# twice154/ofa-for-super-resolution

Hardware: AMD Instinct MI355X
Metric: sr_training_images_per_sec_4x_64to256 (higher is better)
Workload: dtype bf16; 1 GPU; OFA-SR S4 supernet 4x progressive shrinking (elastic kernel {3,5,7}, e=6, d=4, pd=2), LR 64x64 -> HR 256x256, fwd+bwd+Adam, train-mode BN; kernel_transform_mode=1, compat_reference_indexing=True, parallelism=dp1, per_gpu_batch=16, global_batch=16, grad_allreduce_bytes=0, launch=eager

## Files before the change

### ofa-for-super-resolution_amd/csrc/dwconv.hip

```cpp
#include "ofasr_common.h"

#include <type_traits>

namespace ofasr {

constexpr int DW_WAVES = 4;

template <int D>
__device__ __forceinline__ float lane_shift(float v, int lane) {
    if (D == 0) return v;
    const int src = lane + D;
    const float t = __shfl(v, src & 63, 64);
    return (src >= 0 && src < 64) ? t : 0.f;
}

template <int K>
struct Strips {
    static constexpr int PAD = K / 2;
    static __host__ __device__ int count(int W) { return W <= 64 ? 1 : (W + (64 - 2 * PAD) - 1) / (64 - 2 * PAD); }
    static __device__ int col0(int W, int s) { return W <= 64 ? 0 : s * (64 - 2 * PAD) - PAD; }
    static __device__ bool core(int W, int lane) { return W <= 64 ? true : (lane >= PAD && lane < 64 - PAD); }
};

template <typename T, int K, bool FLIP>
__global__ void __launch_bounds__(64 * DW_WAVES) dw_strip_kernel(const T* __restrict__ x, const float* __restrict__ f,
                                                                 T* __restrict__ y, int C, int H, int W,
                                                                 int nstrips, int nchunks, int rows_per_chunk,
                                                                 long long units) {
    constexpr int PAD = K / 2;
    const int lane = lane_id();
    const int wave = __builtin_amdgcn_readfirstlane((int)(threadIdx.x >> 6));
    const long long unit = (long long)blockIdx.x * DW_WAVES + wave;
    if (unit >= units) return;
    const int chunk = (int)(unit % nchunks);
// ... 201 lines not shown

template <typename T, int K> struct VecPx { static constexpr int N = (K <= 3 && sizeof(T) == 2) ? 8 : 4; };

template <int PXL, int PAD>
__device__ __forceinline__ void build_window(const float* v, float* win, int lane, bool has_left, bool has_right) {
#pragma unroll
    for (int i = 0; i < PAD; ++i) {
        const float l = __shfl(v[PXL - PAD + i], (lane + 63) & 63, 64);
        const float r = __shfl(v[i], (lane + 1) & 63, 64);
        win[i] = has_left ? l : 0.f;
        win[PAD + PXL + i] = has_right ? r : 0.f;
    }
#pragma unroll
    for (int i = 0; i < PXL; ++i) win[PAD + i] = v[i];
}

typedef __attribute__((ext_vector_type(16))) float dwm_f32x16;
typedef __attribute__((ext_vector_type(8))) short dwm_s16x8;
typedef __attribute__((ext_vector_type(8))) __bf16 dwm_bf16x8;
typedef __attribute__((ext_vector_type(8))) _Float16 dwm_f16x8;
template <typename T> struct DwMma;
template <> struct DwMma<bf16_t> {
    static __device__ __forceinline__ dwm_f32x16 run(dwm_s16x8 a, dwm_s16x8 b, dwm_f32x16 c) {
        return __builtin_amdgcn_mfma_f32_32x32x16_bf16(__builtin_bit_cast(dwm_bf16x8, a), __builtin_bit_cast(dwm_bf16x8, b),
                                                       c, 0, 0, 0);
    }
};
template <> struct DwMma<f16_t> {
    static __device__ __forceinline__ dwm_f32x16 run(dwm_s16x8 a, dwm_s16x8 b, dwm_f32x16 c) {
        return __builtin_amdgcn_mfma_f32_32x32x16_f16(__builtin_bit_cast(dwm_f16x8, a), __builtin_bit_cast(dwm_f16x8, b), c,
                                                      0, 0, 0);
    }
};
constexpr int DWM_NPW = 4;
constexpr int DWM_PITCH = 144;
__device__ __forceinline__ void dwm_lds_fence() { asm volatile("s_waitcnt lgkmcnt(0)" ::: "memory"); }

template <typename T, int K, bool FLIP, bool XF, bool STAT, bool BX = false>
__global__ void __launch_bounds__(64 * DW_WAVES) dw_mfma_kernel(const T* __restrict__ x, const float* __restrict__ f,
                                                                T* __restrict__ y, int N, int C, int H, int W,
                                                                int nslabs, InputXf xf, StatOut so, BnFold fold,
                                                                BwdXf bx = BwdXf{}) {
    constexpr int PAD = K / 2;
    constexpr int LROWS = 64 + 2 * PAD;
    __shared__ __attribute__((aligned(16))) char planes[DW_WAVES][LROWS * DWM_PITCH];
    __shared__ __attribute__((aligned(16))) char outs[DW_WAVES][64 * 128];
    __shared__ uint16_t tapt[DW_WAVES][K][96];
    const int lane = lane_id();
    const int wave = __builtin_amdgcn_readfirstlane((int)(threadIdx.x >> 6));
    const long long unit = (long long)blockIdx.x * DW_WAVES + wave;
    const int c = (int)(unit % C);
    const int n0 = (int)(unit / C) * DWM_NPW;
    if (n0 >= N) return;
    char* L = planes[wave];
    const int r = lane & 31, hh = lane >> 5;

    for (int i = lane; i < LROWS * (DWM_PITCH / 16); i += 64) *reinterpret_cast<uint4*>(L + i * 16) = make_uint4(0, 0, 0, 0);
    for (int i = lane; i < K * 96; i += 64) tapt[wave][i / 96][i % 96] = 0;
    dwm_lds_fence();
    for (int e = lane; e < K * K; e += 64)
        tapt[wave][e / K][e % K + 40] = from_float<T>(f[(long long)c * K * K + (FLIP ? (K * K - 1 - e) : e)]).v;
    dwm_lds_fence();
    dwm_s16x8 Bf[K][3];
#pragma unroll
    for (int ky = 0; ky < K; ++ky)
#pragma unroll
        for (int ch = 0; ch < 3; ++ch) {
            const int base = (-8 + 16 * ch) + 8 * hh - r + PAD + 40;
            dwm_s16x8 b;
#pragma unroll
            for (int i = 0; i < 8; ++i) b[i] = (short)tapt[wave][ky][base + i];
            Bf[ky][ch] = b;
        }

    float xsc = 1.f, xmu = 0.f, xb = 0.f;
    if constexpr (XF) {
        if (fold.cp) {
            double s = 0.0, ss = 0.0;
            for (int q0 = lane; q0 < fold.P; q0 += 8 * 64) {
                float2 v[8];
#pragma unroll
                for (int j = 0; j < 8; ++j) {
                    const int q = q0 + 64 * j < fold.P ? q0 + 64 * j : fold.P - 1;
                    v[j] = fold.cp[(long long)c * fold.P + q];
                }
#pragma unroll
                for (int j = 0; j < 8; ++j) {
                    const bool live = q0 + 64 * j < fold.P;
                    s += live ? (double)v[j].x : 0.0;
                    ss += live ? (double)v[j].y : 0.0;
                }
            }
#pragma unroll
            for (int o = 32; o > 0; o >>= 1) {
                s += __shfl_xor(s, o, 64);
                ss += __shfl_xor(ss, o, 64);
            }
            const double mean = s / fold.M;
            double var = ss / fold.M - mean * mean;
            var = var < 0.0 ? 0.0 : var;
            const double invstd = 1.0 / sqrt(var + fold.eps);
            const double gm = fold.gamma ? (double)fold.gamma[c] : 1.0, bt = fold.beta ? (double)fold.beta[c] : 0.0;
            xsc = (float)(gm * invstd);
            xmu = (float)mean;
            xb = (float)bt;
            if (n0 == 0 && lane == 0) {
                fold.mean[c] = (float)mean;
                fold.invstd[c] = (float)invstd;
                fold.scale[c] = xsc;
                fold.shift[c] = (float)(bt - mean * gm * invstd);
                if (fold.running_mean) {
                    const double unb = fold.M > 1.0 ? var * fold.M / (fold.M - 1.0) : var;
                    fold.running_mean[c] =
                        (float)((1.0 - fold.momentum) * (double)fold.running_mean[c] + fold.momentum * mean);
                    fold.running_var[c] = (float)((1.0 - fold.momentum) * (double)fold.running_var[c] + fold.momentum * unb);
                }
                if (c == 0) {
#pragma unroll
                    for (int i = 0; i < 3; ++i)
                        if (fold.counters[i]) *fold.counters[i] += 1;
                }
            }
        } else {
            xsc = xf.scale[c];
            xmu = xf.mean[c];
            xb = fmaf(xmu, xsc, xf.shift[c]);
        }
    }

    float bmu = 0.f, bsc = 1.f, bxb = 0.f, bka = 0.f, bkbi = 0.f;
    if constexpr (BX) {
        bmu = bx.mean[c];
        bsc = bx.scale[c];
        bxb = fmaf(bmu, bsc, bx.shift[c]);
        if (bx.fold_partial) bwdxf_fold(bx, c, bsc, n0 == 0 && lane == 0, bka, bkbi);
        else {
            bka = bx.ka[c];
            bkbi = bx.kbi[c];
        }
    }

    int abase[2][3];
#pragma unroll
    for (int wb = 0; wb < 2; ++wb)
#pragma unroll
        for (int ch = 0; ch < 3; ++ch) {
            const int cidx = 4 * wb - 1 + 2 * ch + hh;
            const int cz = (cidx < 0 || cidx >= (W >> 3)) ? 8 : cidx;
            abase[wb][ch] = r * DWM_PITCH + cz * 16;
        }
    const int cpr = W >> 3;
    const int nchunks = H * cpr;
    char* O = outs[wave];
    uint4 nxt[8];
    uint4 nxt2[BX ? 8 : 1];
    auto load_plane = [&](int pl) {
        const long long plane = (long long)(n0 + pl) * C + c;
        const uint4* src = reinterpret_cast<const uint4*>(x + plane * (long long)H * W);
#pragma unroll
        for (int it = 0; it < 8; ++it) {
            const int idx = lane + 64 * it;
            nxt[it] = src[idx < nchunks ? idx : 0];
        }
        if constexpr (BX) {
            const uint4* src2 = reinterpret_cast<const uint4*>(reinterpret_cast<const T*>(bx.y) + plane * (long long)H * W);
#pragma unroll
            for (int it = 0; it < 8; ++it) {
                const int idx = lane + 64 * it;
                nxt2[it] = src2[idx < nchunks ? idx : 0];
            }
        }
    };
    load_plane(0);
    for (int pl = 0; pl < DWM_NPW && n0 + pl < N; ++pl) {
        const long long plane = (long long)(n0 + pl) * C + c;
#pragma unroll
        for (int it = 0; it < 8; ++it) {
            const int idx = lane + 64 * it;
            if (idx < nchunks) {
                uint4 v = nxt[it];
                if constexpr (XF) {
                    uint32_t wv[4] = {v.x, v.y, v.z, v.w};
#pragma unroll
                    for (int i = 0; i < 4; ++i) {
                        T lo, hi;
                        lo.v = (uint16_t)(wv[i] & 0xffffu);
                        hi.v = (uint16_t)(wv[i] >> 16);
                        const float a = fminf(fmaxf(fmaf(to_float(lo) - xmu, xsc, xb), 0.f), 6.f);
                        const float b = fminf(fmaxf(fmaf(to_float(hi) - xmu, xsc, xb), 0.f), 6.f);
                        wv[i] = pack2<T>(a, b);
                    }
                    v = make_uint4(wv[0], wv[1], wv[2], wv[3]);
                }
                if constexpr (BX) {
                    uint32_t wv[4] = {v.x, v.y, v.z, v.w};
                    const uint32_t yv[4] = {nxt2[it].x, nxt2[it].y, nxt2[it].z, nxt2[it].w};
#pragma unroll
                    for (int i = 0; i < 4; ++i) {
                        T lo, hi, ylo, yhi;
                        lo.v = (uint16_t)(wv[i] & 0xffffu);
                        hi.v = (uint16_t)(wv[i] >> 16);
                        ylo.v = (uint16_t)(yv[i] & 0xffffu);
                        yhi.v = (uint16_t)(yv[i] >> 16);
                        const float t0 = to_float(ylo) - bmu, t1 = to_float(yhi) - bmu;
                        const float p0 = fmaf(t0, bsc, bxb), p1 = fmaf(t1, bsc, bxb);
                        const float z0 = (p0 > 0.f && p0 < 6.f) ? to_float(lo) : 0.f;
                        const float z1 = (p1 > 0.f && p1 < 6.f) ? to_float(hi) : 0.f;
                        wv[i] = pack2<T>(fmaf(-t0, bkbi, fmaf(bsc, z0, -bka)), fmaf(-t1, bkbi, fmaf(bsc, z1, -bka)));
                    }
                    v = make_uint4(wv[0], wv[1], wv[2], wv[3]);
                    if (bx.dy_out)
                        reinterpret_cast<uint4*>(reinterpret_cast<T*>(bx.dy_out) + plane * (long long)H * W)[idx] = v;
                }
                const int row = idx / cpr, chunk = idx - row * cpr, lr = row + PAD;
                *reinterpret_cast<uint4*>(L + lr * DWM_PITCH + (chunk << 4)) = v;
            }
        }
        dwm_lds_fence();
        if (pl + 1 < DWM_NPW && n0 + pl + 1 < N) load_plane(pl + 1);
        float st_s = 0.f, st_q = 0.f;
        for (int hb = 0; hb < H / 32; ++hb) {
            const char* Lh = L + hb * (32 * DWM_PITCH);
#pragma unroll
            for (int wb = 0; wb < 2; ++wb) {
                if (32 * wb >= W) break;
                dwm_f32x16 acc;
#pragma unroll
                for (int i = 0; i < 16; ++i) acc[i] = 0.f;
#pragma unroll
                for (int ky = 0; ky < K; ++ky) {
#pragma unroll
                    for (int ch = 0; ch < 3; ++ch) {
                        const dwm_s16x8 a =
                            *reinterpret_cast<const dwm_s16x8*>(Lh + abase[wb][ch] + ky * DWM_PITCH);
                        acc = DwMma<T>::run(Bf[ky][ch], a, acc);
                    }
                }
                const int h = 32 * hb + r;
#pragma unroll
                for (int q = 0; q < 4; ++q) {
                    const uint2 o = make_uint2(pack2<T>(acc[4 * q], acc[4 * q + 1]), pack2<T>(acc[4 * q + 2], acc[4 * q + 3]));
                    const int chunk = 4 * wb + q;
                    *reinterpret_cast<uint2*>(O + h * 128 + ((chunk ^ ((h >> 1) & 7)) << 4) + 8 * hh) = o;
                    if constexpr (STAT) {
                        const uint32_t wv2[2] = {o.x, o.y};
#pragma unroll
                        for (int i = 0; i < 2; ++i) {
                            T lo, hi;
                            lo.v = (uint16_t)(wv2[i] & 0xffffu);
                            hi.v = (uint16_t)(wv2[i] >> 16);
                            const float a0 = to_float(lo), a1 = to_float(hi);
                            st_s += a0 + a1;
                            st_q = fmaf(a0, a0, fmaf(a1, a1, st_q));
                        }
                    }
                }
            }
        }
        dwm_lds_fence();
        uint4* dst = reinterpret_cast<uint4*>(y + plane * (long long)H * W);
#pragma unroll
        for (int it = 0; it < 8; ++it) {
            const int idx = lane + 64 * it;
            if (idx < nchunks) {
                const int row = idx / cpr, chunk = idx - row * cpr;
                dst[idx] = *reinterpret_cast<const uint4*>(O + row * 128 + ((chunk ^ ((row >> 1) & 7)) << 4));
            }
        }
        dwm_lds_fence();
        if constexpr (STAT) {
            const float s = wave_sum(st_s), q = wave_sum(st_q);
            if (lane == 0) {
                so.partial[(long long)c * so.P + (long long)(n0 + pl) * nslabs] = make_float2(s, q);
                for (int sl = 1; sl < nslabs; ++sl)
                    so.partial[(long long)c * so.P + (long long)(n0 + pl) * nslabs + sl] = make_float2(0.f, 0.f);
            }
        }
    }
}

static bool mfma_geom_ok(int64_t H, int64_t W, int K, const void* a, const void* b) {
    const uintptr_t bits = reinterpret_cast<uintptr_t>(a) | reinterpret_cast<uintptr_t>(b);
    return K >= 5 && (W == 32 || W == 64) && H >= 32 && H <= 64 && (H % 32) == 0 && (bits & 15) == 0;
}

struct VecGeom {
    int G, gpw, R, nslabs;
};

template <typename T, int K, bool FLIP, bool XF = false, bool STAT = false, bool BX = false>
__global__ void __launch_bounds__(64 * DW_WAVES) dw_vec_kernel(const T* __restrict__ x, const float* __restrict__ f,
                                                               T* __restrict__ y, int C, int H, int W, VecGeom vg,
                                                               long long nwaves, InputXf xf = InputXf{},
                                                               StatOut so = StatOut{nullptr, 0}, BnFold fold = BnFold{},
                                                               BwdXf bx = BwdXf{}) {
    constexpr int PAD = K / 2;
    constexpr int PXL = VecPx<T, K>::N;
    typedef PxIO<T, PXL> IO;
    typedef typename IO::raw_t raw_t;
    const int lane = lane_id();
    const int wave = __builtin_amdgcn_readfirstlane((int)(threadIdx.x >> 6));
    const long long wunit = (long long)blockIdx.x * DW_WAVES + wave;
    if (wunit >= nwaves) return;
    const int slab = (int)(wunit % vg.nslabs);
    const long long plane = wunit / vg.nslabs;
    const int c = (int)(plane % C);

    float taps[K * K];
#pragma unroll
    for (int e = 0; e < K * K; ++e) taps[e] = f[(long long)c * K * K + (FLIP ? (K * K - 1 - e) : e)];
    float bmu = 0.f, bsc = 1.f, bxb = 0.f, bka = 0.f, bkbi = 0.f;
    if constexpr (BX) {
        bmu = bx.mean[c];
        bsc = bx.scale[c];
        bxb = fmaf(bmu, bsc, bx.shift[c]);
        if (bx.fold_partial) bwdxf_fold(bx, c, bsc, plane < C && slab == 0 && lane == 0, bka, bkbi);
// ... 271 lines not shown
    vg.G = (int)(W / PXL);
    vg.gpw = 64 / vg.G;
    int64_t R = cdiv(H, vg.gpw);
    if (R < 4) R = 4;
    if (R > 32) R = 32;
    vg.R = (int)R;
    vg.nslabs = (int)cdiv(H, (int64_t)vg.gpw * vg.R);
    return true;
}

__global__ void __launch_bounds__(256) dw_wgrad_reduce_kernel(const float* __restrict__ part_out,
                                                              float* __restrict__ df, int nparts, long long CKK) {
    const long long idx = (long long)blockIdx.x * blockDim.x + threadIdx.x;
    if (idx >= CKK) return;
    float s = 0.f;
    for (int p = 0; p < nparts; ++p) s += part_out[(long long)p * CKK + idx];
    df[idx] = s;
}

static int wgrad_parts(int64_t N, int64_t C) {
    int64_t want = cdiv(6144, C > 0 ? C : 1);
    if (want < 1) want = 1;
    if (want > N) want = N;
    return (int)want;
}

template <typename T, bool FLIP, bool XF = false, bool STAT = false, bool BX = false>
static int launch_conv(const char* name, const void* x, const float* f, void* y, int64_t N, int64_t C, int64_t H,
                       int64_t W, int K, hipStream_t st, InputXf xf = InputXf{}, StatOut so = StatOut{nullptr, 0},
                       BnFold fold = BnFold{}, BwdXf bx = BwdXf{}) {
    prof_note(2.0 * sizeof(T) * (double)N * (double)C * (double)H * (double)W + 4.0 * (double)C * K * K,
              2.0 * K * K * (double)N * (double)C * (double)H * (double)W);
    if constexpr (sizeof(T) == 2) {
        if (mfma_geom_ok(H, W, K, x, y)) {
            VecGeom vg0;
            const int nslabs = vec_geom(H, W, 2, 4, x, y, vg0) ? vg0.nslabs : 1;
            if (STAT && so.P != (int)(N * nslabs)) {
                set_error("%s: statistics slab count %d != %lld", name, so.P, (long long)(N * nslabs));
                return OFASR_ERR_INVALID_ARG;
            }
            const long long units = (long long)C * cdiv(N, DWM_NPW);
            if (K == 5)
                OFASR_LAUNCH((dw_mfma_kernel<T, 5, FLIP, XF, STAT, BX>), dim3((unsigned)cdiv(units, DW_WAVES)),
                                   dim3(64 * DW_WAVES), 0, st, (const T*)x, f, (T*)y, (int)N, (int)C, (int)H, (int)W, nslabs,
                                   xf, so, fold, bx);
            else
                OFASR_LAUNCH((dw_mfma_kernel<T, 7, FLIP, XF, STAT, BX>), dim3((unsigned)cdiv(units, DW_WAVES)),
                                   dim3(64 * DW_WAVES), 0, st, (const T*)x, f, (T*)y, (int)N, (int)C, (int)H, (int)W, nslabs,
                                   xf, so, fold, bx);
            return check_launch(name);
        }
    }
    {
        VecGeom vg;
#define OFASR_DWV(KK)                                                                                               \
    if (vec_geom(H, W, (int)sizeof(T), VecPx<T, KK>::N, x, y, vg)) {                                               \
        const long long nwaves = (long long)N * C * vg.nslabs;                                                     \
        if (STAT && so.P != (int)(N * vg.nslabs)) {                                                                \
            set_error("%s: statistics slab count %d != %lld", name, so.P, (long long)(N * vg.nslabs));             \
            return OFASR_ERR_INVALID_ARG;                                                                          \
        }                                                                                                          \
        OFASR_LAUNCH((dw_vec_kernel<T, KK, FLIP, XF, STAT, BX>), dim3((unsigned)cdiv(nwaves, DW_WAVES)),     \
                           dim3(64 * DW_WAVES), 0, st, (const T*)x, f, (T*)y, (int)C, (int)H, (int)W, vg, nwaves,  \
                           xf, so, fold, bx);                                                                      \
        return check_launch(name);                                                                                 \
    }
        switch (K) {
            case 1: OFASR_DWV(1) break;
            case 3: OFASR_DWV(3) break;
            case 5: OFASR_DWV(5) break;
            default: OFASR_DWV(7) break;
        }
#undef OFASR_DWV
    }
    if constexpr (XF || BX) {
        set_error("%s: fused input transform needs the vector kernel", name);
        return OFASR_ERR_UNSUPPORTED;
    }
    const int rows_per_chunk = H <= 32 ? (int)H : 32;
    const int nchunks = (int)cdiv(H, rows_per_chunk);
#define OFASR_DW_LAUNCH(KK)                                                                                  \
    {                                                                                                        \
// ... 435 lines not shown
```

### ofa-for-super-resolution_amd/csrc/conv2d.hip

```cpp
#include "ofasr_common.h"

namespace ofasr {

typedef __attribute__((ext_vector_type(16))) float cv_f32x16;
typedef __attribute__((ext_vector_type(8))) __bf16 cv_bf16x8;
typedef __attribute__((ext_vector_type(8))) _Float16 cv_f16x8;
typedef __attribute__((ext_vector_type(8))) short cv_s16x8;

constexpr int CV_TW = 64;
constexpr int CV_SEG = 20;
constexpr int CV_RP = 4 * CV_SEG;
constexpr int CV_KC = 32;

template <typename T> struct CvMma;
template <> struct CvMma<bf16_t> {
    static __device__ __forceinline__ cv_f32x16 run(cv_s16x8 a, cv_s16x8 b, cv_f32x16 c) {
        return __builtin_amdgcn_mfma_f32_32x32x16_bf16(__builtin_bit_cast(cv_bf16x8, a), __builtin_bit_cast(cv_bf16x8, b),
                                                       c, 0, 0, 0);
    }
};
template <> struct CvMma<f16_t> {
    static __device__ __forceinline__ cv_f32x16 run(cv_s16x8 a, cv_s16x8 b, cv_f32x16 c) {
        return __builtin_amdgcn_mfma_f32_32x32x16_f16(__builtin_bit_cast(cv_f16x8, a), __builtin_bit_cast(cv_f16x8, b), c,
                                                      0, 0, 0);
    }
};

__device__ __forceinline__ int cv_pos(int r, int col) { return r * CV_RP + (col & 3) * CV_SEG + (col >> 2); }
__device__ __forceinline__ int cv_rec(int P, int j) { return P * 64 + ((j ^ ((P >> 2) & 3)) << 4); }

struct CvBn {
    float* ss;
    const float* gamma;
// ... 476 lines not shown
    const int wq = wave % (WCO * WCI);
    if constexpr (WK > 1) {
        static_assert(WCO * WCI * RBW * 4096 <= ROWS * 256, "Yt holds one tx slice per (wco, wci)");
        float* red = reinterpret_cast<float*>(Yt) + wq * (RBW * 16 * 64) + lane;
#pragma unroll
        for (int tx = 0; tx < KS; ++tx) {
#pragma unroll
            for (int ph = 1; ph < WK; ++ph) {
                __syncthreads();
                if (wk == ph) {
#pragma unroll
                    for (int rb = 0; rb < RBW; ++rb)
#pragma unroll
                        for (int reg = 0; reg < 16; ++reg) red[(rb * 16 + reg) * 64] = acc[rb][tx][reg];
                }
                __syncthreads();
                if (wk == 0) {
#pragma unroll
                    for (int rb = 0; rb < RBW; ++rb)
#pragma unroll
                        for (int reg = 0; reg < 16; ++reg) acc[rb][tx][reg] += red[(rb * 16 + reg) * 64];
                }
            }
        }
        if (wk != 0) return;
    }
    float* dst = part + ((((long long)split * KS + ty) * P.nz + z) * (WCO * WCI) + wq) * (RBW * KS * 16 * 64) + lane;
#pragma unroll
    for (int rb = 0; rb < RBW; ++rb)
#pragma unroll
        for (int tx = 0; tx < KS; ++tx)
#pragma unroll
            for (int reg = 0; reg < 16; ++reg) dst[((rb * KS + tx) * 16 + reg) * 64] = acc[rb][tx][reg];
}

template <int KS, int RBW, int WCO, int WCI>
__global__ void __launch_bounds__(256) conv_wgrad_reduce_kernel(const float* __restrict__ part, float* __restrict__ dw,
                                                                CvWgParams P, long long total) {
    const long long idx = (long long)blockIdx.x * blockDim.x + threadIdx.x;
    if (idx >= total) return;
    constexpr int PER_WAVE = RBW * KS * 16 * 64;
    long long t = idx;
    const int lane = (int)(t & 63);
    t >>= 6;
    const int reg = (int)(t & 15);
    t >>= 4;
    const int tx = (int)(t % KS);
    t /= KS;
    const int rb = (int)(t % RBW);
    t /= RBW;
    const int wq = (int)(t % (WCO * WCI));
    t /= (WCO * WCI);
    const int z = (int)(t % P.nz);
    const int ty = (int)(t / P.nz);
    const int wco = wq % WCO, wci = wq / WCO;
    const int coslab = z / P.ncislab, cislab = z % P.ncislab;
    const int co = coslab * (32 * RBW * WCO) + 32 * (wco * RBW + rb) + (reg & 3) + 8 * (reg >> 2) + 4 * (lane >> 5);
    const int ci = cislab * (32 * WCI) + 32 * wci + (lane & 31);
    if (co >= P.Cout || ci >= P.Cin) return;
    const long long inner = ((long long)(rb * KS + tx) * 16 + reg) * 64 + lane;
    float sum = 0.f;
    const long long sstride = (long long)KS * P.nz * (WCO * WCI) * PER_WAVE;
    const float* src = part + (((long long)ty * P.nz + z) * (WCO * WCI) + wq) * PER_WAVE + inner;
    for (int split = 0; split < P.ksplit; ++split) sum += src[split * sstride];
    dw[(((long long)co * P.Cin + ci) * KS + ty) * KS + tx] = sum;
}
// ... 7 lines not shown
};

static CvWgPlan cv_wg_plan(int64_t N, int64_t Cin, int64_t Cout, int64_t H, int64_t W, int K) {
    CvWgPlan p{};
    p.note_bytes = 2.0 * (double)N * (double)H * (double)W * (double)(Cin + Cout);
    p.note_flops = 2.0 * (double)N * (double)H * (double)W * (double)Cin * (double)Cout * K * K;
    const bool wide = Cin > 32;
    const int rcls = Cout > 64 ? 0 : (Cout > 32 ? 1 : 2);
    p.cfg = (wide ? 0 : 3) + rcls;
    p.rows = rcls == 0 ? 128 : (rcls == 1 ? 64 : 32);
    p.rbw = rcls == 2 ? 1 : 2;
    p.cib = wide ? 64 : 32;
    CvWgParams& P = p.P;
    P.Cin = (int)Cin; P.Cout = (int)Cout; P.H = (int)H; P.W = (int)W;
    P.tiles_x = (int)cdiv(W, CV_TW); P.tiles_y = (int)cdiv(H, 2);
    P.ntiles = (int)(N * P.tiles_x * P.tiles_y);
    P.ncislab = (int)cdiv(Cin, p.cib);
    P.nz = (int)cdiv(Cout, p.rows) * P.ncislab;
    int ks = 512 / (K * P.nz);
    ks = ks > P.ntiles / 8 ? P.ntiles / 8 : ks;
    if (ks > 8) ks -= ks % 8;
    P.ksplit = ks < 1 ? 1 : ks;
    const int nwq = wide ? (rcls == 0 ? 4 : 2) : (rcls == 0 ? 2 : 1);
    p.part_bytes = (size_t)P.ksplit * K * P.nz * nwq * (p.rbw * K * 16 * 64) * sizeof(float);
    return p;
}

template <typename T>
static int launch_conv2d_wgrad(const char* name, const void* dy, const void* x, float* dw, int K, const CvWgPlan& p, void* ws,
                               hipStream_t st) {
    const CvWgParams& P = p.P;
    dim3 grid((unsigned)(cdiv(P.ksplit, 8) * 8 * K * P.nz));
    prof_note(p.note_bytes, p.note_flops);
#define OFASR_WG(KS, RBW, WCO, WCI, WK)                                                                              \
    {                                                                                                                \
        OFASR_LAUNCH((conv_wgrad_kernel<T, KS, RBW, WCO, WCI, WK>), grid, dim3(256), 0, st, (const T*)dy,      \
                           (const T*)x, (float*)ws, P);                                                              \
        int rc = check_launch(name);                                                                                 \
        if (rc) return rc;                                                                                           \
        const long long tot = (long long)KS * P.nz * (WCO * WCI) * RBW * KS * 16 * 64;                               \
        OFASR_LAUNCH((conv_wgrad_reduce_kernel<KS, RBW, WCO, WCI>), dim3((unsigned)cdiv(tot, 256)),            \
                           dim3(256), 0, st, (const float*)ws, dw, P, tot);                                          \
    }
#define OFASR_WGK(KS)                                                                                                \
    switch (p.cfg) {                                                                                                 \
        case 0: OFASR_WG(KS, 2, 2, 2, 1) break;                                                                      \
        case 1: OFASR_WG(KS, 2, 1, 2, 2) break;                                                                      \
        case 2: OFASR_WG(KS, 1, 1, 2, 2) break;                                                                      \
        case 3: OFASR_WG(KS, 2, 2, 1, 2) break;                                                                      \
        case 4: OFASR_WG(KS, 2, 1, 1, 4) break;                                                                      \
        default: OFASR_WG(KS, 1, 1, 1, 4) break;                                                                     \
    }
    if (K == 5) { OFASR_WGK(5) } else { OFASR_WGK(3) }
#undef OFASR_WGK
#undef OFASR_WG
    return check_launch(name);
}

static int conv_stat_units(int64_t N, int64_t Cin, int64_t Cout, int64_t H, int64_t W, int K) {
    if (conv_thin_out_supported(Cout, Cin, K, W, OFASR_BF16, nullptr, nullptr))
        return conv_thin_out_units(N, Cout, Cin, H, W, OFASR_BF16);
    if (conv_thin_in_supported(Cin, Cout, K, W, OFASR_BF16, nullptr, nullptr))
        return conv_thin_in_units(N, Cin, Cout, H, W, OFASR_BF16);
    const CvPlan p = cv_plan(Cin, Cout, K, 0, N, H, W);
    const int wp = p.th / 2;
    return (int)(N * cdiv(W, CV_TW) * cdiv(H, p.th) * wp);
}
// ... 155 lines not shown
```

Measured before the change: 2789 images/s.

## Adapt depthwise MFMA conv planes-per-wave to CU count with channel-contiguous work split

Replaces the fixed four-images-per-wave assignment of the MFMA depthwise conv with a plan that picks planes-per-wave from the CU count, so small N*C launches fill the GPU. Waves now walk a contiguous range of (channel, image) planes and may cross channels, so per-channel setup (taps, BN fold statistics, backward fold) moves into a re-entrant routine. That routine issues its global loads early and prefetches the first plane before the LDS setup. It also adds a waves-per-EU hint and an environment override. The cost is redundant per-channel fold reductions across more waves and more complex counter and writer logic.

New measurement: 2754 images/s. 0.987x the previous value.

```diff
diff --git a/ofa-for-super-resolution_amd/csrc/dw_fill.h b/ofa-for-super-resolution_amd/csrc/dw_fill.h
--- /dev/null
+++ b/ofa-for-super-resolution_amd/csrc/dw_fill.h
@@ -0,0 +1,55 @@
+#pragma once
+
+#if defined(__HIPCC__)
+#define OFASR_DWF_HD __host__ __device__ __forceinline__
+#else
+#define OFASR_DWF_HD inline
+#endif
+
+namespace ofasr {
+
+constexpr int DWF_MAX_PPW = 4;
+constexpr int DWF_WAVES_PER_SIMD = 2;
+constexpr int DWF_SIMDS_PER_CU = 4;
+
+struct DwFill {
+    int ppw;
+    int legacy;
+};
+
+OFASR_DWF_HD long long dwf_waves(int N, int C, DwFill pl) {
+    if (pl.legacy) return (long long)C * ((N + DWF_MAX_PPW - 1) / DWF_MAX_PPW);
+    return ((long long)N * C + pl.ppw - 1) / pl.ppw;
+}
+
+OFASR_DWF_HD void dwf_range(long long u, int N, int C, DwFill pl, int& p0, int& p1) {
+    const long long total = (long long)N * C;
+    long long a, b;
+    if (pl.legacy) {
+        const long long c = u % C, n0 = (u / C) * DWF_MAX_PPW;
+        a = c * N + (n0 < N ? n0 : N);
+        b = c * N + (n0 + DWF_MAX_PPW < N ? n0 + DWF_MAX_PPW : N);
+    } else {
+        a = u * pl.ppw;
+        b = a + pl.ppw;
+    }
+    if (u < 0 || a > total) a = total;
+    if (u < 0 || b > total) b = total;
+    p0 = (int)a;
+    p1 = (int)b;
+}
+
+OFASR_DWF_HD int dwf_channel(int p, int N) { return p / N; }
+OFASR_DWF_HD int dwf_image(int p, int N) { return p % N; }
+OFASR_DWF_HD bool dwf_is_writer(int p, int N) { return p % N == 0; }
+OFASR_DWF_HD bool dwf_owns_counters(int p) { return p == 0; }
+
+inline int dwf_choose_ppw(long long planes, long long slots) {
+    for (int ppw = 1; ppw < DWF_MAX_PPW; ++ppw)
+        if ((planes + ppw - 1) / ppw <= slots) return ppw;
+    return DWF_MAX_PPW;
+}
+
+inline long long dwf_slots(int cu_count) { return (long long)DWF_WAVES_PER_SIMD * DWF_SIMDS_PER_CU * cu_count; }
+
+}
diff --git a/ofa-for-super-resolution_amd/csrc/dwconv.hip b/ofa-for-super-resolution_amd/csrc/dwconv.hip
--- a/ofa-for-super-resolution_amd/csrc/dwconv.hip
+++ b/ofa-for-super-resolution_amd/csrc/dwconv.hip
@@ -1,5 +1,9 @@
 #include "ofasr_common.h"
-
+#include "dw_fill.h"
+
+#include <string.h>
+
+#include <atomic>
 #include <type_traits>
 
 namespace ofasr {
@@ -267,15 +271,14 @@
                                                       0, 0, 0);
     }
 };
-constexpr int DWM_NPW = 4;
 constexpr int DWM_PITCH = 144;
 __device__ __forceinline__ void dwm_lds_fence() { asm volatile("s_waitcnt lgkmcnt(0)" ::: "memory"); }
 
 template <typename T, int K, bool FLIP, bool XF, bool STAT, bool BX = false>
-__global__ void __launch_bounds__(64 * DW_WAVES) dw_mfma_kernel(const T* __restrict__ x, const float* __restrict__ f,
+__global__ void __launch_bounds__(64 * DW_WAVES) __attribute__((amdgpu_waves_per_eu(2))) dw_mfma_kernel(const T* __restrict__ x, const float* __restrict__ f,
                                                                 T* __restrict__ y, int N, int C, int H, int W,
-                                                                int nslabs, InputXf xf, StatOut so, BnFold fold,
-                                                                BwdXf bx = BwdXf{}) {
+                                                                int nslabs, DwFill plan, InputXf xf, StatOut so,
+                                                                BnFold fold, BwdXf bx = BwdXf{}) {
     constexpr int PAD = K / 2;
     constexpr int LROWS = 64 + 2 * PAD;
     __shared__ __attribute__((aligned(16))) char planes[DW_WAVES][LROWS * DWM_PITCH];
@@ -283,36 +286,120 @@
     __shared__ uint16_t tapt[DW_WAVES][K][96];
     const int lane = lane_id();
     const int wave = __builtin_amdgcn_readfirstlane((int)(threadIdx.x >> 6));
-    const long long unit = (long long)blockIdx.x * DW_WAVES + wave;
-    const int c = (int)(unit % C);
-    const int n0 = (int)(unit / C) * DWM_NPW;
-    if (n0 >= N) return;
+    int p0, p1;
+    dwf_range((long long)blockIdx.x * DW_WAVES + wave, N, C, plan, p0, p1);
+    if (p0 >= p1) return;
     char* L = planes[wave];
     const int r = lane & 31, hh = lane >> 5;
 
-    for (int i = lane; i < LROWS * (DWM_PITCH / 16); i += 64) *reinterpret_cast<uint4*>(L + i * 16) = make_uint4(0, 0, 0, 0);
-    for (int i = lane; i < K * 96; i += 64) tapt[wave][i / 96][i % 96] = 0;
-    dwm_lds_fence();
-    for (int e = lane; e < K * K; e += 64)
-        tapt[wave][e / K][e % K + 40] = from_float<T>(f[(long long)c * K * K + (FLIP ? (K * K - 1 - e) : e)]).v;
-    dwm_lds_fence();
+    int abase[2][3];
+#pragma unroll
+    for (int wb = 0; wb < 2; ++wb)
+#pragma unroll
+        for (int ch = 0; ch < 3; ++ch) {
+            const int cidx = 4 * wb - 1 + 2 * ch + hh;
+            const int cz = (cidx < 0 || cidx >= (W >> 3)) ? 8 : cidx;
+            abase[wb][ch] = r * DWM_PITCH + cz * 16;
+        }
+    const int cpr = W >> 3;
+    const int nchunks = H * cpr;
+    char* O = outs[wave];
+    uint4 nxt[8];
+    uint4 nxt2[BX ? 8 : 1];
+    auto load_plane = [&](int p) {
+        const long long plane = (long long)dwf_image(p, N) * C + dwf_channel(p, N);
+        const uint4* src = reinterpret_cast<const uint4*>(x + plane * (long long)H * W);
+        int ll = lane;
+        asm volatile("" : "+v"(ll));
+#pragma unroll
+        for (int it = 0; it < 8; ++it) {
+            const int idx = ll + 64 * it;
+            nxt[it] = src[idx < nchunks ? idx : 0];
+        }
+        if constexpr (BX) {
+            const uint4* src2 = reinterpret_cast<const uint4*>(reinterpret_cast<const T*>(bx.y) + plane * (long long)H * W);
+#pragma unroll
+            for (int it = 0; it < 8; ++it) {
+                const int idx = ll + 64 * it;
+                nxt2[it] = src2[idx < nchunks ? idx : 0];
+            }
+        }
+    };
     dwm_s16x8 Bf[K][3];
-#pragma unroll
-    for (int ky = 0; ky < K; ++ky)
-#pragma unroll
-        for (int ch = 0; ch < 3; ++ch) {
-            const int base = (-8 + 16 * ch) + 8 * hh - r + PAD + 40;
-            dwm_s16x8 b;
-#pragma unroll
-            for (int i = 0; i < 8; ++i) b[i] = (short)tapt[wave][ky][base + i];
-            Bf[ky][ch] = b;
-        }
-
     float xsc = 1.f, xmu = 0.f, xb = 0.f;
+    float bmu = 0.f, bsc = 1.f, bxb = 0.f, bka = 0.f, bkbi = 0.f;
+    constexpr bool EARLY = !BX;
+    auto enter_channel = [&](const int c, const bool writer, const bool counters, const bool first, const int p_first) {
+    static_assert(K * K <= 64, "one tap per lane");
+    int ln = lane;
+    asm volatile("" : "+v"(ln));
+    const int te = ln < K * K ? ln : 0;
+    const float tapv = f[(long long)c * K * K + (FLIP ? (K * K - 1 - te) : te)];
+    float2 v0[8];
+    float gmv = 1.f, btv = 0.f, rmv = 0.f, rvv = 0.f;
+    long long cnt[3] = {0, 0, 0};
+    if constexpr (XF) {
+        if (fold.cp) {
+#pragma unroll
+            for (int j = 0; j < 8; ++j) {
+                const int q = ln + 64 * j < fold.P ? ln + 64 * j : fold.P - 1;
+                v0[j] = fold.cp[(long long)c * fold.P + q];
+            }
+            if (fold.gamma) gmv = fold.gamma[c];
+            if (fold.beta) btv = fold.beta[c];
+            if (fold.running_mean) {
+                rmv = fold.running_mean[c];
+                rvv = fold.running_var[c];
+            }
+            if (counters) {
+#pragma unroll
+                for (int i = 0; i < 3; ++i)
+                    if (fold.counters[i]) cnt[i] = *fold.counters[i];
+            }
+        } else {
+            xsc = xf.scale[c];
+            xmu = xf.mean[c];
+            xb = xf.shift[c];
+        }
+    }
+    double fa[8], fb[8];
+    float bsh = 0.f, binv = 0.f;
+    if constexpr (BX) {
+        bmu = bx.mean[c];
+        bsc = bx.scale[c];
+        bsh = bx.shift[c];
+        if (bx.fold_partial) {
+            binv = bx.fold_invstd[c];
+#pragma unroll
+            for (int j = 0; j < 8; ++j) {
+                const int q = j < bx.fold_P ? j : bx.fold_P - 1;
+                fa[j] = bx.fold_partial[((long long)q * bx.fold_C + c) * 2];
+                fb[j] = bx.fold_partial[((long long)q * bx.fold_C + c) * 2 + 1];
+            }
+        } else {
+            bka = bx.ka[c];
+            bkbi = bx.kbi[c];
+        }
+    }
+    if constexpr (EARLY)
+        if (first) load_plane(p_first);
+    __builtin_amdgcn_sched_barrier(0);
+
+    if (first) {
+        for (int i = ln; i < LROWS * (DWM_PITCH / 16); i += 64) *reinterpret_cast<uint4*>(L + i * 16) = make_uint4(0, 0, 0, 0);
+        for (int i = ln; i < K * 96; i += 64) tapt[wave][i / 96][i % 96] = 0;
+        dwm_lds_fence();
+    }
     if constexpr (XF) {
         if (fold.cp) {
             double s = 0.0, ss = 0.0;
-            for (int q0 = lane; q0 < fold.P; q0 += 8 * 64) {
+#pragma unroll
+            for (int j = 0; j < 8; ++j) {
+                const bool live = ln + 64 * j < fold.P;
+                s += live ? (double)v0[j].x : 0.0;
+                ss += live ? (double)v0[j].y : 0.0;
+            }
+            for (int q0 = ln + 8 * 64; q0 < fold.P; q0 += 8 * 64) {
                 float2 v[8];
 #pragma unroll
                 for (int j = 0; j < 8; ++j) {
@@ -335,80 +422,92 @@
             double var = ss / fold.M - mean * mean;
             var = var < 0.0 ? 0.0 : var;
             const double invstd = 1.0 / sqrt(var + fold.eps);
-            const double gm = fold.gamma ? (double)fold.gamma[c] : 1.0, bt = fold.beta ? (double)fold.beta[c] : 0.0;
+            const double gm = fold.gamma ? (double)gmv : 1.0, bt = fold.beta ? (double)btv : 0.0;
             xsc = (float)(gm * invstd);
             xmu = (float)mean;
             xb = (float)bt;
-            if (n0 == 0 && lane == 0) {
+            if (writer && lane == 0) {
                 fold.mean[c] = (float)mean;
                 fold.invstd[c] = (float)invstd;
                 fold.scale[c] = xsc;
                 fold.shift[c] = (float)(bt - mean * gm * invstd);
                 if (fold.running_mean) {
                     const double unb = fold.M > 1.0 ? var * fold.M / (fold.M - 1.0) : var;
-                    fold.running_mean[c] =
-                        (float)((1.0 - fold.momentum) * (double)fold.running_mean[c] + fold.momentum * mean);
-                    fold.running_var[c] = (float)((1.0 - fold.momentum) * (double)fold.running_var[c] + fold.momentum * unb);
-                }
-                if (c == 0) {
+                    fold.running_mean[c] = (float)((1.0 - fold.momentum) * (double)rmv + fold.momentum * mean);
+                    fold.running_var[c] = (float)((1.0 - fold.momentum) * (double)rvv + fold.momentum * unb);
+                }
+                if (counters) {
 #pragma unroll
                     for (int i = 0; i < 3; ++i)
-                        if (fold.counters[i]) *fold.counters[i] += 1;
+                        if (fold.counters[i]) {
+                            long long bump = 1;
+                            for (int j = 0; j < i; ++j) bump += fold.counters[j] == fold.counters[i] ? 1 : 0;
+                            *fold.counters[i] = cnt[i] + bump;
+                        }
                 }
             }
         } else {
-            xsc = xf.scale[c];
-            xmu = xf.mean[c];
-            xb = fmaf(xmu, xsc, xf.shift[c]);
-        }
-    }
-
-    float bmu = 0.f, bsc = 1.f, bxb = 0.f, bka = 0.f, bkbi = 0.f;
+            xb = fmaf(xmu, xsc, xb);
+        }
+    }
+
     if constexpr (BX) {
-        bmu = bx.mean[c];
-        bsc = bx.scale[c];
-        bxb = fmaf(bmu, bsc, bx.shift[c]);
-        if (bx.fold_partial) bwdxf_fold(bx, c, bsc, n0 == 0 && lane == 0, bka, bkbi);
-        else {
-            bka = bx.ka[c];
-            bkbi = bx.kbi[c];
-        }
-    }
-
-    int abase[2][3];
-#pragma unroll
-    for (int wb = 0; wb < 2; ++wb)
+        bxb = fmaf(bmu, bsc, bsh);
+        if (bx.fold_partial) {
+            double s = 0.0, sx = 0.0;
+            asm volatile("" : "+v"(s), "+v"(sx), "+v"(binv));
+#pragma unroll
+            for (int j = 0; j < 8; ++j) {
+                s += j < bx.fold_P ? fa[j] : 0.0;
+                sx += j < bx.fold_P ? fb[j] : 0.0;
+            }
+            for (int q0 = 8; q0 < bx.fold_P; q0 += 8) {
+#pragma unroll
+                for (int j = 0; j < 8; ++j) {
+                    const int q = q0 + j < bx.fold_P ? q0 + j : bx.fold_P - 1;
+                    fa[j] = bx.fold_partial[((long long)q * bx.fold_C + c) * 2];
+                    fb[j] = bx.fold_partial[((long long)q * bx.fold_C + c) * 2 + 1];
+                }
+#pragma unroll
+                for (int j = 0; j < 8; ++j) {
+                    s += q0 + j < bx.fold_P ? fa[j] : 0.0;
+                    sx += q0 + j < bx.fold_P ? fb[j] : 0.0;
+                }
+            }
+            bka = bx.fold_training ? (float)((double)bsc * (s / bx.fold_M)) : 0.f;
+            bkbi = bx.fold_training ? (float)((double)bsc * (double)binv * (sx / bx.fold_M)) : 0.f;
+            if (writer && lane == 0) {
+                if (bx.fold_dgamma) bx.fold_dgamma[c] = (float)sx;
+                if (bx.fold_dbeta) bx.fold_dbeta[c] = (float)s;
+                if (bx.coef_ka) bx.coef_ka[c] = bka;
+                if (bx.coef_kbi) bx.coef_kbi[c] = bkbi;
+            }
+        }
+    }
+
+    if (ln < K * K) tapt[wave][ln / K][ln % K + 40] = from_float<T>(tapv).v;
+    dwm_lds_fence();
+#pragma unroll
+    for (int ky = 0; ky < K; ++ky)
 #pragma unroll
         for (int ch = 0; ch < 3; ++ch) {
-            const int cidx = 4 * wb - 1 + 2 * ch + hh;
-            const int cz = (cidx < 0 || cidx >= (W >> 3)) ? 8 : cidx;
-            abase[wb][ch] = r * DWM_PITCH + cz * 16;
-        }
-    const int cpr = W >> 3;
-    const int nchunks = H * cpr;
-    char* O = outs[wave];
-    uint4 nxt[8];
-    uint4 nxt2[BX ? 8 : 1];
-    auto load_plane = [&](int pl) {
-        const long long plane = (long long)(n0 + pl) * C + c;
-        const uint4* src = reinterpret_cast<const uint4*>(x + plane * (long long)H * W);
-#pragma unroll
-        for (int it = 0; it < 8; ++it) {
-            const int idx = lane + 64 * it;
-            nxt[it] = src[idx < nchunks ? idx : 0];
-        }
-        if constexpr (BX) {
-            const uint4* src2 = reinterpret_cast<const uint4*>(reinterpret_cast<const T*>(bx.y) + plane * (long long)H * W);
-#pragma unroll
-            for (int it = 0; it < 8; ++it) {
-                const int idx = lane + 64 * it;
-                nxt2[it] = src2[idx < nchunks ? idx : 0];
-            }
-        }
+            const int base = (-8 + 16 * ch) + 8 * (ln >> 5) - (ln & 31) + PAD + 40;
+            dwm_s16x8 b;
+#pragma unroll
+            for (int i = 0; i < 8; ++i) b[i] = (short)tapt[wave][ky][base + i];
+            Bf[ky][ch] = b;
+        }
+    dwm_lds_fence();
     };
-    load_plane(0);
-    for (int pl = 0; pl < DWM_NPW && n0 + pl < N; ++pl) {
-        const long long plane = (long long)(n0 + pl) * C + c;
+
+    for (int p = p0; p < p1;) {
+        const int c = dwf_channel(p, N);
+        const int pe = min(p1, (c + 1) * N);
+        enter_channel(c, dwf_is_writer(p, N), dwf_owns_counters(p), p == p0, p);
+        if constexpr (!EARLY) load_plane(p);
+    for (; p < pe; ++p) {
+        const int n = dwf_image(p, N);
+        const long long plane = (long long)n * C + c;
 #pragma unroll
         for (int it = 0; it < 8; ++it) {
             const int idx = lane + 64 * it;
@@ -452,7 +551,7 @@
             }
         }
         dwm_lds_fence();
-        if (pl + 1 < DWM_NPW && n0 + pl + 1 < N) load_plane(pl + 1);
+        if (p + 1 < (EARLY ? p1 : pe)) load_plane(p + 1);
         float st_s = 0.f, st_q = 0.f;
         for (int hb = 0; hb < H / 32; ++hb) {
             const char* Lh = L + hb * (32 * DWM_PITCH);
@@ -506,17 +605,40 @@
         if constexpr (STAT) {
             const float s = wave_sum(st_s), q = wave_sum(st_q);
             if (lane == 0) {
-                so.partial[(long long)c * so.P + (long long)(n0 + pl) * nslabs] = make_float2(s, q);
+                so.partial[(long long)c * so.P + (long long)n * nslabs] = make_float2(s, q);
                 for (int sl = 1; sl < nslabs; ++sl)
-                    so.partial[(long long)c * so.P + (long long)(n0 + pl) * nslabs + sl] = make_float2(0.f, 0.f);
-            }
-        }
+                    so.partial[(long long)c * so.P + (long long)n * nslabs + sl] = make_float2(0.f, 0.f);
+            }
+        }
+    }
     }
 }
 
 static bool mfma_geom_ok(int64_t H, int64_t W, int K, const void* a, const void* b) {
     const uintptr_t bits = reinterpret_cast<uintptr_t>(a) | reinterpret_cast<uintptr_t>(b);
     return K >= 5 && (W == 32 || W == 64) && H >= 32 && H <= 64 && (H % 32) == 0 && (bits & 15) == 0;
+}
+
+static DwFill dw_fill_plan(long long planes) {
+    static const int forced = [] {
+        const char* e = getenv("OFASR_DW_MFMA_PPW");
+        if (!e || !e[0]) return 0;
+        if (!strcmp(e, "legacy")) return -1;
+        return (e[0] >= '1' && e[0] <= '0' + DWF_MAX_PPW && !e[1]) ? e[0] - '0' : 0;
+    }();
+    if (forced < 0) return DwFill{DWF_MAX_PPW, 1};
+    if (forced > 0) return DwFill{forced, 0};
+    constexpr int MAXDEV = 64;
+    static std::atomic<int> cus[MAXDEV];
+    int dev = 0, n = 0;
+    if (hipGetDevice(&dev) != hipSuccess || dev < 0 || dev >= MAXDEV) return DwFill{DWF_MAX_PPW, 0};
+    n = cus[dev].load(std::memory_order_relaxed);
+    if (n == 0) {
+        if (hipDeviceGetAttribute(&n, hipDeviceAttributeMultiprocessorCount, dev) != hipSuccess || n <= 0)
+            return DwFill{DWF_MAX_PPW, 0};
+        cus[dev].store(n, std::memory_order_relaxed);
+    }
+    return DwFill{dwf_choose_ppw(planes, dwf_slots(n)), 0};
 }
 
 struct VecGeom {
@@ -854,22 +976,23 @@
     prof_note(2.0 * sizeof(T) * (double)N * (double)C * (double)H * (double)W + 4.0 * (double)C * K * K,
               2.0 * K * K * (double)N * (double)C * (double)H * (double)W);
     if constexpr (sizeof(T) == 2) {
-        if (mfma_geom_ok(H, W, K, x, y)) {
+        if (mfma_geom_ok(H, W, K, x, y) && N * C <= INT32_MAX) {
             VecGeom vg0;
             const int nslabs = vec_geom(H, W, 2, 4, x, y, vg0) ? vg0.nslabs : 1;
             if (STAT && so.P != (int)(N * nslabs)) {
                 set_error("%s: statistics slab count %d != %lld", name, so.P, (long long)(N * nslabs));
                 return OFASR_ERR_INVALID_ARG;
             }
-            const long long units = (long long)C * cdiv(N, DWM_NPW);
+            const DwFill plan = dw_fill_plan(N * C);
+            const long long units = dwf_waves((int)N, (int)C, plan);
             if (K == 5)
                 OFASR_LAUNCH((dw_mfma_kernel<T, 5, FLIP, XF, STAT, BX>), dim3((unsigned)cdiv(units, DW_WAVES)),
                                    dim3(64 * DW_WAVES), 0, st, (const T*)x, f, (T*)y, (int)N, (int)C, (int)H, (int)W, nslabs,
-                                   xf, so, fold, bx);
+                                   plan, xf, so, fold, bx);
             else
                 OFASR_LAUNCH((dw_mfma_kernel<T, 7, FLIP, XF, STAT, BX>), dim3((unsigned)cdiv(units, DW_WAVES)),
                                    dim3(64 * DW_WAVES), 0, st, (const T*)x, f, (T*)y, (int)N, (int)C, (int)H, (int)W, nslabs,
-                                   xf, so, fold, bx);
+                                   plan, xf, so, fold, bx);
             return check_launch(name);
         }
     }
```

## Add warp-specialized double-buffered conv weight-gradient kernel with async LDS loads

Applied to the files above, without the earlier changes.

Adds a new conv weight-gradient kernel that splits each block into four compute waves running MFMA and four loader waves. The loader waves fill double-buffered LDS tiles, dy through global_load_lds DMA and x through register transpose with swizzled stores. The goal is to overlap global memory loads with matrix math and to feed B fragments through ds_read_tr instead of the older kernel's staging. It runs only for cfg 0 with K of 3 or 5, suitable shapes and 16-byte aligned inputs, can be turned off with an env var, and adds an extra reduce kernel and a 512-thread block at occupancy 1.

Result: no change. 2791 images/s before, 2808 images/s after (median of 6 runs) (+0.6%).

```diff
diff --git a/ofa-for-super-resolution_amd/csrc/conv2d.hip b/ofa-for-super-resolution_amd/csrc/conv2d.hip
--- a/ofa-for-super-resolution_amd/csrc/conv2d.hip
+++ b/ofa-for-super-resolution_amd/csrc/conv2d.hip
@@ -1,4 +1,5 @@
 #include "ofasr_common.h"
+#include "conv_wgrad_pipe.h"
 
 namespace ofasr {
 
@@ -541,6 +542,151 @@
         for (int tx = 0; tx < KS; ++tx)
 #pragma unroll
             for (int reg = 0; reg < 16; ++reg) dst[((rb * KS + tx) * 16 + reg) * 64] = acc[rb][tx][reg];
+}
+
+__device__ __forceinline__ void cwp_dma16(const void* src, char* lds_piece) {
+    __builtin_amdgcn_global_load_lds((const __attribute__((address_space(1))) void*)src,
+                                     (__attribute__((address_space(3))) void*)lds_piece, 16, 0, 0);
+}
+__device__ __forceinline__ void cwp_barrier() { asm volatile("s_waitcnt vmcnt(0) lgkmcnt(0)\n\ts_barrier" ::: "memory"); }
+
+template <typename T, int KS>
+__global__ void __launch_bounds__(CWP_THREADS, 1) conv_wgrad_pipe_kernel(const T* __restrict__ dy, const T* __restrict__ x,
+                                                                         float* __restrict__ part, CvWgParams P) {
+    constexpr int PAD = KS / 2;
+    constexpr int RBW = 2, WCO = 2;
+    constexpr int REC = CWP_REC, XW = CWP_XW;
+    __shared__ __attribute__((aligned(1024))) char lds[CWP_LDS_BYTES];
+
+    const int G = KS * P.nz;
+    const int xcd = blockIdx.x & 7, jb = blockIdx.x >> 3;
+    const int group = jb % G, split = (jb / G) * 8 + xcd;
+    if (split >= P.ksplit) return;
+    const int ty = group % KS, z = group / KS;
+    const int coslab = z / P.ncislab, cislab = z % P.ncislab;
+    const int lane = lane_id();
+    const int wave = __builtin_amdgcn_readfirstlane((int)(threadIdx.x >> 6));
+    const int t0 = cwp_split_begin(split, P.ksplit, P.ntiles), ntl = cwp_split_begin(split + 1, P.ksplit, P.ntiles) - t0;
+
+    if (wave < CWP_COMPUTE_WAVES) {
+        const int wco = wave % WCO, wci = wave / WCO;
+        const int c = lane & 31, h = lane >> 5;
+        const int g = lane >> 4, q = (lane >> 2) & 3, pp = lane & 3;
+        int xbase[2][2];
+        {
+            const int L = 8 * (g >> 1) + q;
+            const int cb = 64 * wci + 32 * (g & 1) + 8 * pp;
+#pragma unroll
+            for (int b1 = 0; b1 < 2; ++b1)
+#pragma unroll
+                for (int b0 = 0; b0 < 2; ++b0) {
+                    const int bit1 = ((L >> 1) & 1) ^ b1 ^ (b0 & L & 1);
+                    xbase[b1][b0] = L * 128 + ((wci ^ bit1) << 6) + (cb & 63);
+                }
+        }
+        int aoff[RBW];
+#pragma unroll
+        for (int rb = 0; rb < RBW; ++rb) aoff[rb] = 32 * (wco * RBW + rb) + c;
+        cv_f32x16 acc[RBW][KS];
+#pragma unroll
+        for (int rb = 0; rb < RBW; ++rb)
+#pragma unroll
+            for (int tx = 0; tx < KS; ++tx)
+#pragma unroll
+                for (int i = 0; i < 16; ++i) acc[rb][tx][i] = 0.f;
+        cwp_barrier();
+        for (int i = 0; i < ntl; ++i) {
+            const char* Yt = lds + cwp_yt_off(i & 1);
+            const char* Xt = lds + cwp_xt_off(i & 1);
+#pragma unroll
+            for (int s = 0; s < 8; ++s) {
+                cv_s16x8 A[RBW];
+#pragma unroll
+                for (int rb = 0; rb < RBW; ++rb)
+                    A[rb] = *reinterpret_cast<const cv_s16x8*>(Yt + cwp_yfrag_off(aoff[rb], 2 * s + h));
+#pragma unroll
+                for (int tx = 0; tx < KS; ++tx) {
+                    const int Da = (s >> 2) * XW + 16 * (s & 3) + 8 - PAD + tx, Db = Da + 4;
+                    const cv_s16x4 lo = __builtin_amdgcn_ds_read_tr16_b64_v4i16(
+                        (cv_lds_s16x4*)(Xt + xbase[(Da >> 1) & 1][Da & 1] + Da * REC));
+                    const cv_s16x4 hi = __builtin_amdgcn_ds_read_tr16_b64_v4i16(
+                        (cv_lds_s16x4*)(Xt + xbase[(Db >> 1) & 1][Db & 1] + Db * REC));
+                    const cv_s16x8 B = __builtin_shufflevector(lo, hi, 0, 1, 2, 3, 4, 5, 6, 7);
+#pragma unroll
+                    for (int rb = 0; rb < RBW; ++rb) acc[rb][tx] = CvMma<T>::run(A[rb], B, acc[rb][tx]);
+                }
+            }
+            cwp_barrier();
+        }
+        float* dst = part + ((((long long)split * KS + ty) * P.nz + z) * 4 + wave) * (RBW * KS * 16 * 64) + lane;
+#pragma unroll
+        for (int rb = 0; rb < RBW; ++rb)
+#pragma unroll
+            for (int tx = 0; tx < KS; ++tx)
+#pragma unroll
+                for (int reg = 0; reg < 16; ++reg) dst[((rb * KS + tx) * 16 + reg) * 64] = acc[rb][tx][reg];
+    } else {
+        const int lw = wave - CWP_COMPUTE_WAVES;
+        const int lt = (int)threadIdx.x - 64 * CWP_COMPUTE_WAVES;
+        const long long HW = (long long)P.H * P.W;
+        const CwpXTask xk = cwp_xtask(lt);
+        const bool xwave = 64 * lw < CWP_XTASKS, xlive = lt < CWP_XTASKS;
+        const int prow = cwp_piece_row(cwp_piece_of(lw, 0), lane), pchunk = cwp_piece_chunk(cwp_piece_of(lw, 0), lane);
+        auto fill = [&](int tile, int b) {
+            const CwpTile t = cwp_tile(tile, P.tiles_x, P.tiles_y);
+            char* Yt = lds + cwp_yt_off(b);
+            char* Xt = lds + cwp_xt_off(b);
+            uint4 v[8];
+            uint32_t okm[8];
+            if (xwave) {
+                const T* xn = x + (long long)t.n * P.Cin * HW;
+                const int gy = t.ty0 + xk.r + ty - PAD, gx = t.tx0 - 8 + 8 * xk.run;
+                const bool inb = xlive && gy >= 0 && gy < P.H && gx >= 0 && gx < P.W;
+                const int cbase = cislab * CWP_CIB + 8 * xk.cg;
+#pragma unroll
+                for (int i = 0; i < 8; ++i) {
+                    const bool ok = inb && cbase + i < P.Cin;
+                    okm[i] = ok ? 0xffffffffu : 0u;
+                    v[i] = *reinterpret_cast<const uint4*>(xn + (ok ? ((long long)(cbase + i) * P.H + gy) * P.W + gx : 0));
+                }
+            }
+            {
+                const T* src = dy + cwp_dy_elem(t, coslab * CWP_ROWS + prow, pchunk, P.Cout, P.H, P.W);
+#pragma unroll
+                for (int k = 0; k < CWP_PPW; ++k)
+                    cwp_dma16(src + (long long)(4 * CWP_LOADER_WAVES * k) * HW, Yt + cwp_piece_of(lw, k) * CWP_PIECE_BYTES);
+            }
+            if (xwave) {
+#pragma unroll
+                for (int i = 0; i < 8; ++i) {
+                    v[i].x &= okm[i]; v[i].y &= okm[i]; v[i].z &= okm[i]; v[i].w &= okm[i];
+                }
+#pragma unroll
+                for (int k = 0; k < 4; ++k) {
+                    uint32_t lo[4], hi[4];
+#pragma unroll
+                    for (int m = 0; m < 4; ++m) {
+                        const uint32_t a = k == 0 ? v[2 * m].x : k == 1 ? v[2 * m].y : k == 2 ? v[2 * m].z : v[2 * m].w;
+                        const uint32_t b2 = k == 0 ? v[2 * m + 1].x : k == 1 ? v[2 * m + 1].y : k == 2 ? v[2 * m + 1].z
+                                                                                                       : v[2 * m + 1].w;
+                        lo[m] = __builtin_amdgcn_perm(b2, a, 0x05040100u);
+                        hi[m] = __builtin_amdgcn_perm(b2, a, 0x07060302u);
+                    }
+                    const int R = cwp_xrec(xk, k);
+                    if (xlive) {
+                        *reinterpret_cast<uint4*>(Xt + cwp_xoff(R, xk.cg)) = make_uint4(lo[0], lo[1], lo[2], lo[3]);
+                        *reinterpret_cast<uint4*>(Xt + cwp_xoff(R + 1, xk.cg)) = make_uint4(hi[0], hi[1], hi[2], hi[3]);
+                    }
+                }
+            }
+        };
+        if (ntl > 0) fill(t0, 0);
+        cwp_barrier();
+        for (int i = 0; i < ntl; ++i) {
+            if (cwp_fills_next(i, ntl)) fill(t0 + i + 1, (i + 1) & 1);
+            cwp_barrier();
+        }
+    }
 }
 
 template <int KS, int RBW, int WCO, int WCI>
@@ -614,7 +760,25 @@
     const CvWgParams& P = p.P;
     dim3 grid((unsigned)(cdiv(P.ksplit, 8) * 8 * K * P.nz));
     prof_note(p.note_bytes, p.note_flops);
-#define OFASR_WG(KS, RBW, WCO, WCI, WK)                                                                              \
+    static const bool pipe_on = [] { const char* e = getenv("OFASR_CONV_WGRAD_PIPE"); return !(e && e[0] == '0'); }();
+    if (pipe_on && p.cfg == 0 && cwp_shape_ok(P.Cin, P.Cout, P.H, P.W) &&
+        ((reinterpret_cast<uintptr_t>(dy) | reinterpret_cast<uintptr_t>(x)) & 15) == 0) {
+        if (K == 5)
+            OFASR_LAUNCH((conv_wgrad_pipe_kernel<T, 5>), grid, dim3(CWP_THREADS), 0, st, (const T*)dy, (const T*)x, (float*)ws, P);
+        else
+            OFASR_LAUNCH((conv_wgrad_pipe_kernel<T, 3>), grid, dim3(CWP_THREADS), 0, st, (const T*)dy, (const T*)x, (float*)ws, P);
+        int rc = check_launch(name);
+        if (rc) return rc;
+        const long long tot = (long long)K * P.nz * 4 * 2 * K * 16 * 64;
+        if (K == 5)
+            OFASR_LAUNCH((conv_wgrad_reduce_kernel<5, 2, 2, 2>), dim3((unsigned)cdiv(tot, 256)), dim3(256), 0, st,
+                         (const float*)ws, dw, P, tot);
+        else
+            OFASR_LAUNCH((conv_wgrad_reduce_kernel<3, 2, 2, 2>), dim3((unsigned)cdiv(tot, 256)), dim3(256), 0, st,
+                         (const float*)ws, dw, P, tot);
+        return check_launch(name);
+    }
+#define OFASR_WG(KS, RBW, WCO, WCI, WK)                                                                             \
     {                                                                                                                \
         OFASR_LAUNCH((conv_wgrad_kernel<T, KS, RBW, WCO, WCI, WK>), grid, dim3(256), 0, st, (const T*)dy,      \
                            (const T*)x, (float*)ws, P);                                                              \
diff --git a/ofa-for-super-resolution_amd/csrc/conv_wgrad_pipe.h b/ofa-for-super-resolution_amd/csrc/conv_wgrad_pipe.h
--- /dev/null
+++ b/ofa-for-super-resolution_amd/csrc/conv_wgrad_pipe.h
@@ -0,0 +1,76 @@
+#pragma once
+#include <stdint.h>
+
+#if defined(__HIPCC__) || defined(__CUDACC__)
+#define CWP_HD __host__ __device__ inline
+#else
+#define CWP_HD inline
+#endif
+
+namespace ofasr {
+
+constexpr int CWP_ROWS = 128;
+constexpr int CWP_CIB = 64;
+constexpr int CWP_REC = 2 * CWP_CIB;
+constexpr int CWP_XW = 80;
+constexpr int CWP_TW = 64;
+constexpr int CWP_YT_BYTES = CWP_ROWS * 256;
+constexpr int CWP_XT_BYTES = 2 * CWP_XW * CWP_REC;
+constexpr int CWP_BUF_BYTES = CWP_YT_BYTES + CWP_XT_BYTES;
+constexpr int CWP_LDS_BYTES = 2 * CWP_BUF_BYTES;
+constexpr int CWP_COMPUTE_WAVES = 4;
+constexpr int CWP_LOADER_WAVES = 4;
+constexpr int CWP_THREADS = 64 * (CWP_COMPUTE_WAVES + CWP_LOADER_WAVES);
+constexpr int CWP_PIECE_BYTES = 1024;
+constexpr int CWP_PIECES = CWP_YT_BYTES / CWP_PIECE_BYTES;
+constexpr int CWP_PPW = CWP_PIECES / CWP_LOADER_WAVES;
+constexpr int CWP_XTASKS = (CWP_CIB / 8) * 2 * 10;
+
+CWP_HD bool cwp_shape_ok(long long Cin, long long Cout, long long H, long long W) {
+    return Cin > 32 && Cout > 64 && Cout % CWP_ROWS == 0 && H % 2 == 0 && W % CWP_TW == 0;
+}
+
+CWP_HD int cwp_yt_off(int b) { return b * CWP_BUF_BYTES; }
+CWP_HD int cwp_xt_off(int b) { return b * CWP_BUF_BYTES + CWP_YT_BYTES; }
+
+CWP_HD int cwp_yfrag_off(int row, int chunk) { return row * 256 + ((chunk ^ (row & 15)) << 4); }
+CWP_HD int cwp_piece_of(int lw, int k) { return lw + CWP_LOADER_WAVES * k; }
+CWP_HD int cwp_piece_lds(int piece, int lane) { return piece * CWP_PIECE_BYTES + lane * 16; }
+CWP_HD int cwp_piece_row(int piece, int lane) { return 4 * piece + (lane >> 4); }
+CWP_HD int cwp_piece_chunk(int piece, int lane) { return (lane & 15) ^ (cwp_piece_row(piece, lane) & 15); }
+
+struct CwpTile {
+    int n, ty0, tx0;
+};
+CWP_HD CwpTile cwp_tile(int tile, int tiles_x, int tiles_y) {
+    const int tpi = tiles_x * tiles_y;
+    CwpTile t;
+    t.n = tile / tpi;
+    const int trem = tile - t.n * tpi;
+    t.ty0 = (trem / tiles_x) * 2;
+    t.tx0 = (trem % tiles_x) * CWP_TW;
+    return t;
+}
+
+CWP_HD long long cwp_dy_elem(const CwpTile& t, int co, int chunk, int Cout, int H, int W) {
+    return (((long long)t.n * Cout + co) * H + (t.ty0 + (chunk >> 3))) * W + t.tx0 + 8 * (chunk & 7);
+}
+
+struct CwpXTask {
+    int run, r, cg;
+};
+CWP_HD CwpXTask cwp_xtask(int lt) {
+    CwpXTask k;
+    k.run = lt % 10;
+    k.r = (lt / 10) & 1;
+    k.cg = lt / 20;
+    return k;
+}
+CWP_HD int cwp_xoff(int R, int chunk) { return R * 128 + ((((chunk >> 2) ^ ((R >> 1) & 1))) << 6) + ((chunk & 3) << 4); }
+CWP_HD int cwp_xrec(const CwpXTask& k, int step) { return k.r * CWP_XW + 8 * k.run + 2 * step; }
+
+CWP_HD int cwp_split_begin(int split, int ksplit, int ntiles) { return (int)((long long)split * ntiles / ksplit); }
+CWP_HD bool cwp_fills_next(int i, int ntl) { return i + 1 < ntl; }
+CWP_HD int cwp_barriers(int ntl) { return 1 + (ntl > 0 ? ntl : 0); }
+
+}
```
